# acg-team/ProGraphMSA

Hardware: AMD Instinct MI355X
Metric: DP cell-updates/sec (GCUPS) + wall-clock on 256 seqs × 1000 aa, WAG (higher is better)
Workload: dtype f32

## Files before the change

prographmsa_amd/csrc/pgm_align_kernels.h:

```cpp
#ifndef PGM_ALIGN_KERNELS_H_
#define PGM_ALIGN_KERNELS_H_

#include <hip/hip_runtime.h>
#include <math.h>
#include <type_traits>
#include "pgm_device.h"

#define PGM_NEG_INF (-INFINITY)

__device__ __forceinline__ float pgm_ls_log_add(float x, float add) {
    const float a = 2.44247459618085927548717403238913328776812604856113966238617812902399112761292613763080658235564f;
    const float b = -4.2040783745848554315883301529007786406310628696382695994938550046831869207082846248658671f;
    const float c = -0.72123729809042963774358701619456664388406302428056983119308906451199556380646306f;
    const uint32_t bits = __float_as_uint(x);
    const float e = (float)((int32_t)(bits >> 23) - 126);
    const float d = __uint_as_float(((bits << 9) >> 9) ^ 0x3f000000u);
    float t = __fdiv_rn(b, __fsub_rn(d, c));
    const float u = __fadd_rn(e, a);
    t = __fadd_rn(t, add);
    t = __fadd_rn(t, u);
    return t;
}

__device__ __forceinline__ float pgm_emission_finish(float num, float ay, float bx, float match_init) {
    float q = __fdiv_rn(num, __fmul_rn(ay, bx));
    if (q != q) q = __uint_as_float(0xFFC00000u);
    return pgm_ls_log_add(q, match_init);
}

template <int DMAX, int NODES>
__global__ void __launch_bounds__(NODES) pgm_prep_kernel(const PgmJob *__restrict__ jobs, int *__restrict__ sync, uint32_t sync_ints) {
    extern __shared__ float prep_lds[];
    {
        const uint32_t nthreads = gridDim.x * gridDim.y * gridDim.z * NODES;
        const uint32_t gid = ((blockIdx.z * gridDim.y + blockIdx.y) * gridDim.x + blockIdx.x) * NODES + threadIdx.x;
        for (uint32_t i = gid; i < sync_ints; i += nthreads) sync[i] = 0;
    }
    const PgmJob &J = jobs[blockIdx.x];
    const bool first = blockIdx.y == 0;
    const uint32_t n = first ? J.n1 : J.n2;
    const uint32_t v0 = blockIdx.z * NODES;
    if (v0 >= n) return;
    if (J.tabhdr && J.tabhdr[0] == 0) {
        const uint32_t nc = J.dim + 2u;
        bool any = n - 1u >= v0 && n - 1u < v0 + (uint32_t)NODES;
        for (uint32_t c = 0; c < nc; ++c) {
            const uint32_t r = (uint32_t)J.tabhdr[1u + (first ? 0u : nc) + c];
            any = any || (r != 0u && r - 1u >= v0 && r - 1u < v0 + (uint32_t)NODES);
        }
        if (!any) return;
    }
    const uint32_t D = J.dim, DP = J.dp, ST = D + 1;
    float *Mf = prep_lds;
    float *pif = prep_lds + D * D;
    float *nl = pif + D;
    const uint32_t nn = min((uint32_t)NODES, n - v0);
    {
        const int32_t *pp = first ? J.pp1 : J.pp2;
        const uint32_t *pc = first ? J.pc1 : J.pc2, *pu = first ? J.pu1 : J.pu2;
        const float *pv = first ? J.pv1 : J.pv2;
        PgmTbNode *rec = (first ? J.tb1 : J.tb2) + v0;
        for (uint32_t i = threadIdx.x; i < nn * PGM_TB_PK; i += NODES) {
            const uint32_t node = i / PGM_TB_PK, k = i % PGM_TB_PK;
            const int32_t eb = pp[v0 + node];
            const uint32_t cnt = (uint32_t)(pp[v0 + node + 1] - eb);
            const int32_t e = cnt == 0u ? 0 : eb + (int32_t)min(k, cnt - 1u);
            if (k == 0) rec[node].cnt = cnt;
            rec[node].c[k] = pc[e]; rec[node].v[k] = pv[e]; rec[node].u[k] = pu[e];
        }
    }
    if (!first) for (uint32_t i = threadIdx.x; i < D * D; i += NODES) Mf[i] = (float)J.M[i];
    for (uint32_t i = threadIdx.x; i < D; i += NODES) pif[i] = (float)J.pi[i];
    const double *sites = first ? J.sites1 : J.sites2;
    const uint32_t *smap = first ? J.smap1 : J.smap2;
    float *dst = (first ? J.g1f : J.t2) + (size_t)DP * v0;
    for (uint32_t i = threadIdx.x; i < nn * D; i += NODES) {
        const uint32_t node = v0 + i / D;
        const float g = (float)sites[(size_t)D * (smap ? smap[node] : node) + i % D];
        nl[(i / D) * ST + (i % D)] = g;
        if (first && DP == D) dst[i] = g;
    }
    __syncthreads();
    const uint32_t v = threadIdx.x;
    float g[DMAX];
    float acc = 0.0f;
    if (v < nn) {
#pragma unroll
        for (int k = 0; k < DMAX; ++k) g[k] = ((uint32_t)k < D) ? nl[v * ST + k] : 0.0f;
        float l0 = 0.0f, l1 = 0.0f, l2 = 0.0f, l3 = 0.0f;
        const uint32_t aligned = D / 4u * 4u;
#pragma unroll
        for (int k = 0; k + 3 < DMAX; k += 4) {
            if ((uint32_t)k < aligned) {
                l0 = __fadd_rn(l0, __fmul_rn(g[k], pif[k]));
                l1 = __fadd_rn(l1, __fmul_rn(g[k + 1], pif[k + 1]));
                l2 = __fadd_rn(l2, __fmul_rn(g[k + 2], pif[k + 2]));
                l3 = __fadd_rn(l3, __fmul_rn(g[k + 3], pif[k + 3]));
            }
        }
        acc = __fadd_rn(0.0f, __fadd_rn(__fadd_rn(l0, l2), __fadd_rn(l1, l3)));
#pragma unroll
        for (int k = 0; k < DMAX; ++k)
            if ((uint32_t)k >= aligned && (uint32_t)k < D) acc = __fadd_rn(acc, __fmul_rn(g[k], pif[k]));
        (first ? J.a1 : J.b2)[v0 + v] = acc;
    }
    if (first) {
        if (DP != D && v < nn) {
#pragma unroll
            for (int k = 0; k < DMAX; ++k) if ((uint32_t)k < DP) dst[(size_t)DP * v + k] = g[k];
        }
        return;
    }
    __syncthreads();
    if (v < nn) {
        for (uint32_t k = 0; k < D; ++k) {
            float t = 0.0f;
#pragma unroll
            for (int j = 0; j < DMAX; ++j)
                if ((uint32_t)j < D) t = __fadd_rn(t, __fmul_rn(Mf[j + D * k], g[j]));
            nl[v * ST + k] = t;
        }
    }
    __syncthreads();
    for (uint32_t i = threadIdx.x; i < nn * DP; i += NODES) {
        const uint32_t node = i / DP, k = i % DP;
        dst[i] = k < D ? nl[node * ST + k] : 0.0f;
    }
}

#define PGM_TAB_HDR 136
__global__ void __launch_bounds__(256) pgm_classify_kernel(const PgmJob *__restrict__ jobs) {
    const PgmJob &J = jobs[blockIdx.x];
    if (!J.tabhdr) return;
    const bool first = blockIdx.y == 0;
    const uint32_t n = first ? J.n1 : J.n2, D = J.dim;
    const double *sites = first ? J.sites1 : J.sites2;
    const uint32_t *smap = first ? J.smap1 : J.smap2;
    uint8_t *cls = (uint8_t *)(first ? J.cls1 : J.cls2);
    const float uni = (float)(1.0 / (double)D);
    for (uint32_t v = blockIdx.z * blockDim.x + threadIdx.x; v < n; v += gridDim.z * blockDim.x) {
        const double *col = sites + (size_t)D * (smap ? smap[v] : v);
        uint32_t nz = 0, sym = 0;
        bool same = true;
        float vs = 0.f;
        const float g0 = (float)col[0];
        for (uint32_t k = 0; k < D; ++k) {
            const float g = (float)col[k];
            if (g != 0.0f) { ++nz; sym = k; vs = g; }
            same = same && g == g0;
        }
        uint32_t c = 255u;
        if (nz == 0u) c = D + 1u;
        else if (nz == 1u && vs == 1.0f) c = sym;
        else if (same && g0 == uni) c = D;
        cls[v] = (uint8_t)c;
        if (c == 255u) atomicOr(J.tabhdr, 1);
        else atomicCAS(J.tabhdr + 1 + (first ? 0u : D + 2u) + c, 0, (int)v + 1);
    }
}

__device__ __forceinline__ size_t pgm_cell_index(const PgmJob &J, uint32_t y, uint32_t x) {
    const uint32_t b = y / PGM_ROWS, l = PGM_HALO + (y - b * PGM_ROWS);
    return ((size_t)b * J.tsteps + (x + l)) * 64u + l;
}
__device__ __forceinline__ float4 pgm_load_cell(const PgmJob &J, uint32_t y, uint32_t x) {
    return J.cells[pgm_cell_index(J, y, x)];
}

__device__ __forceinline__ float pgm_dpp_wave_shr1(float src, float lane0_value) {
    return __int_as_float(__builtin_amdgcn_update_dpp(__float_as_int(lane0_value), __float_as_int(src), 0x138, 0xf, 0xf, false));
}

#define PGM_GLOBAL __attribute__((address_space(1)))
typedef float pgm_v4f __attribute__((ext_vector_type(4)));
template <class T> __device__ __forceinline__ T pgm_gld(const T *p) { return *(const PGM_GLOBAL T *)(uintptr_t)p; }
#define PGM_EM_TB 4
template <int DP, int RB>
__global__ void __launch_bounds__(4 * PGM_ROWS) pgm_emission_skew_kernel(const PgmJob *__restrict__ jobs) {
    typedef float pgm_v2f __attribute__((ext_vector_type(2)));
    constexpr int NT = DP / 4;
    constexpr int COLS = 64 + PGM_EM_TB * PGM_BLOCK - PGM_HALO - 1;
    constexpr int STR = DP + 1;
    __shared__ pgm_v2f tp[(COLS + 1) * STR];
    __shared__ float bq[COLS];
    const PgmJob &J = jobs[blockIdx.z];
    const uint32_t tb0 = blockIdx.x * PGM_EM_TB;
    const uint32_t rsh = J.rshift, nvb = J.nb << rsh;
    if (tb0 >= J.nblk || 4u * RB * blockIdx.y >= nvb) return;
    if (J.tabhdr && pgm_gld(J.tabhdr) == 0) return;
    auto row_of = [&](uint32_t v, uint32_t lane_) { return ((((v >> rsh) << 6) + lane_) << rsh) | (v & ((1u << rsh) - 1u)); };
    auto sblock_of = [&](uint32_t v, uint32_t tb_) { return ((((size_t)(v >> rsh) * J.nblk + tb_) << rsh) | (v & ((1u << rsh) - 1u))); };
    const uint32_t t0 = tb0 * PGM_BLOCK;
    const int cbase = (int)t0 - 63;
    if ((DP == 20 || DP == 4) && RB == 1) {
        constexpr int TE = DP + 1;
        float *const tab = (float *)tp;
        static_assert(COLS * TE <= (COLS + 1) * STR * 2, "score table must fit the column staging area");
        static_assert(DP > 20 || TE <= 32, "row classes must fit As");
        __shared__ float As[32];
        const uint32_t fb0 = 4u * blockIdx.y + threadIdx.x / PGM_ROWS;
        const uint32_t fl = threadIdx.x % PGM_ROWS;
        const bool active = fb0 < nvb;
        int sym = DP;
        bool plain = true;
        float a_row = 0.f;
        if (active) {
            const uint32_t y = row_of(fb0, fl);
            const uint32_t yc = (y + 1 < J.n1) ? y : 0u;
            const float4 *src = (const float4 *)(J.g1f + (size_t)DP * yc);
            int nz = 0;
#pragma unroll
            for (int q = 0; q < NT; ++q) {
                const float4 v = src[q];
                const float vv[4] = {v.x, v.y, v.z, v.w};
#pragma unroll
                for (int u = 0; u < 4; ++u)
                    if (vv[u] != 0.0f) { ++nz; sym = 4 * q + u; plain = plain && vv[u] == 1.0f; }
            }
            plain = plain && nz <= 1;
            a_row = J.a1[yc];
        }
        if (threadIdx.x < 32) As[threadIdx.x] = 0.f;
        if (__syncthreads_and(plain ? 1 : 0)) {
            if (active) As[sym] = a_row;
            __syncthreads();
            const float mi = J.sc.match_init;
            constexpr int NE = (COLS * TE + 4 * PGM_ROWS - 1) / (4 * PGM_ROWS);
            float tt[NE], tb2[NE];
#pragma unroll
            for (int e = 0; e < NE; ++e) {
                const int i = (int)threadIdx.x + e * 4 * PGM_ROWS;
                const int ci = i / TE, k = i % TE, c = cbase + ci;
                const bool in = i < COLS * TE && c >= 0 && c <= (int)J.ncol;
                tb2[e] = in ? J.b2[c] : 0.f;
                tt[e] = (in && k < DP) ? J.t2[(size_t)DP * c + k] : 0.f;
            }
#pragma unroll
            for (int e = 0; e < NE; ++e) {
                const int i = (int)threadIdx.x + e * 4 * PGM_ROWS;
                if (i < COLS * TE) tab[i] = pgm_emission_finish(0.0f + tt[e], As[i % TE], tb2[e], mi);
            }
            __syncthreads();
            if (!active) return;
            PGM_GLOBAL pgm_v4f *const Sq = (PGM_GLOBAL pgm_v4f *)(uintptr_t)J.S;
            const int l = PGM_HALO + (int)fl;
#pragma unroll 1
            for (int w = 0; w < PGM_EM_TB; ++w) {
                const uint32_t tb = tb0 + w;
                if (tb >= J.nblk) break;
                float out[PGM_BLOCK];
#pragma unroll
                for (int i = 0; i < PGM_BLOCK; ++i) out[i] = tab[((int)(tb * PGM_BLOCK) + i - l - cbase) * TE + sym];
                PGM_GLOBAL pgm_v4f *dst = Sq + (sblock_of(fb0, tb) * 64u + (uint32_t)l) * (PGM_BLOCK / 4);
#pragma unroll
                for (int q = 0; q < PGM_BLOCK / 4; ++q) dst[q] = pgm_v4f{out[4 * q], out[4 * q + 1], out[4 * q + 2], out[4 * q + 3]};
            }
            return;
        }
    }
    const float4 *t2q = (const float4 *)J.t2;
    float *tpf = (float *)tp;
    for (int i = threadIdx.x; i < (COLS + 1) * NT; i += 4 * PGM_ROWS) {
        const int ci = i / NT, q = i % NT, c = cbase + ci;
        float4 v = make_float4(0.f, 0.f, 0.f, 0.f);
        if (c >= 0 && c <= (int)J.ncol) v = t2q[(size_t)NT * c + q];
        const float vv[4] = {v.x, v.y, v.z, v.w};
#pragma unroll
        for (int u = 0; u < 4; ++u) {
            const int k = 4 * q + u;
            if (ci < COLS) tpf[2 * (ci * STR + k)] = vv[u];
            if (ci > 0) tpf[2 * ((ci - 1) * STR + k) + 1] = vv[u];
        }
    }
    for (int i = threadIdx.x; i < COLS; i += 4 * PGM_ROWS) {
        const int col = cbase + i;
        bq[i] = (col >= 0 && col <= (int)J.ncol) ? J.b2[col] : 0.f;
    }
    __syncthreads();
    const uint32_t b0 = (4u * blockIdx.y + threadIdx.x / PGM_ROWS) * RB;
    const int l = PGM_HALO + (int)(threadIdx.x % PGM_ROWS);
    if (b0 >= nvb) return;
    float gy[RB][DP], ay[RB];
#pragma unroll
    for (int r = 0; r < RB; ++r) {
        const uint32_t y = row_of(b0 + (uint32_t)r, (uint32_t)(l - PGM_HALO));
        const uint32_t yc = (y + 1 < J.n1) ? y : 0u;
        const float4 *src = (const float4 *)(J.g1f + (size_t)DP * yc);
#pragma unroll
        for (int q = 0; q < NT; ++q) {
            const float4 v = src[q];
            gy[r][4 * q] = v.x; gy[r][4 * q + 1] = v.y; gy[r][4 * q + 2] = v.z; gy[r][4 * q + 3] = v.w;
        }
        ay[r] = J.a1[yc];
    }
    const float mi = J.sc.match_init;
    const uint32_t nblk = J.nblk;
    PGM_GLOBAL pgm_v4f *const Sq = (PGM_GLOBAL pgm_v4f *)(uintptr_t)J.S;
#pragma unroll 1
    for (int w = 0; w < PGM_EM_TB; ++w) {
        const uint32_t tb = tb0 + w;
        if (tb >= nblk) break;
        float out[RB][PGM_BLOCK];
#pragma unroll
        for (int i = 0; i < PGM_BLOCK; i += 2) {
            const int ci = (int)(tb * PGM_BLOCK) + i - l - cbase;
            const pgm_v2f *tc = tp + ci * STR;
            pgm_v2f acc[RB];
#pragma unroll
            for (int r = 0; r < RB; ++r) acc[r] = pgm_v2f{0.0f, 0.0f};
#pragma unroll
            for (int k = 0; k < DP; ++k) {
                const pgm_v2f tk = tc[k];
#pragma unroll
                for (int r = 0; r < RB; ++r) {
                    const pgm_v2f g = {gy[r][k], gy[r][k]};
                    acc[r] = acc[r] + g * tk;
                }
            }
#pragma unroll
            for (int r = 0; r < RB; ++r) {
                out[r][i] = pgm_emission_finish(acc[r].x, ay[r], bq[ci], mi);
                out[r][i + 1] = pgm_emission_finish(acc[r].y, ay[r], bq[ci + 1], mi);
            }
        }
#pragma unroll
        for (int r = 0; r < RB; ++r) {
            if (b0 + (uint32_t)r < nvb) {
                PGM_GLOBAL pgm_v4f *dst = Sq + (sblock_of(b0 + (uint32_t)r, tb) * 64u + (uint32_t)l) * (PGM_BLOCK / 4);
#pragma unroll
                for (int q = 0; q < PGM_BLOCK / 4; ++q) dst[q] = pgm_v4f{out[r][4 * q], out[r][4 * q + 1], out[r][4 * q + 2], out[r][4 * q + 3]};
            }
        }
// ... 2263 lines not shown
```

prographmsa_amd/csrc/pgm_capi.hip:

```cpp
#include <hip/hip_runtime.h>

#include <algorithm>
#include <cmath>
#include <cstdio>
#include <thread>
#include <atomic>
#include <chrono>
#include <queue>
#include <cstdlib>
#include <cstring>
#include <numeric>
#include <mutex>
#include <string>
#include <unordered_set>
#include <vector>
#include <sys/mman.h>

#include "pgm_align_kernels.h"
#include "pgm_crit_kernels.h"
#include "pgm_nw_kernels.h"
#include "pgm_csprofile_kernels.h"
#include "pgm_dist_kernels.h"
#include "pgm_merge_kernels.h"
#include "pgm_parsimony_kernels.h"
// ... 88 lines not shown
static hipError_t pinned_alloc(size_t bytes, void **out) {
    const size_t H = (size_t)2 << 20, len = (std::max<size_t>(bytes, 1) + H - 1) / H * H;
    void *p = getenv("PGM_PINNED_MALLOC") ? nullptr : aligned_alloc(H, len);
    if (p) {
        (void)madvise(p, len, MADV_HUGEPAGE);
        (void)lib_pool().run(len / H, len >= 8 * H ? 16u : 1u, [&](size_t c) { for (size_t o = 0; o < H; o += 4096) ((volatile char *)p)[c * H + o] = 0; });
        if (hipHostRegister(p, len, hipHostRegisterDefault) == hipSuccess) {
            std::lock_guard<std::mutex> g(g_pinned_mu);
            g_pinned_registered.insert(p);
            *out = p;
            return hipSuccess;
        }
        (void)hipGetLastError();
        free(p);
    }
    return hipHostMalloc(out, bytes, hipHostMallocDefault);
}
static void pinned_free(void *p) {
    if (!p) return;
    bool reg;
    { std::lock_guard<std::mutex> g(g_pinned_mu); reg = g_pinned_registered.erase(p) != 0; }
    if (reg) { (void)hipHostUnregister(p); free(p); }
    else (void)hipHostFree(p);
}
static void slot_free(int slot, void *p) {
    if (slot == pgm_ctx::C_HIN) pinned_free(p);
    else if (slot == pgm_ctx::C_HOST) (void)hipHostFree(p);
    else (void)hipFree(p);
}

struct pgm_align_batch {
    uint32_t njobs = 0;
    uint64_t cells = 0;
    uint32_t maxdim = 0, maxnb = 0, maxn = 0, maxnblk = 0;
    std::vector<PgmJob> jobs;
    std::vector<uint32_t> order;
    BatchSchedule sched;
    uint8_t *d_in = nullptr;
    uint8_t *d_work = nullptr;
    uint8_t *d_cells = nullptr;
    uint8_t *d_out = nullptr;
    uint8_t *d_S = nullptr;
    uint8_t *d_small = nullptr;
    size_t in_bytes = 0, work_bytes = 0, cell_bytes = 0, out_bytes = 0, s_bytes = 0, small_bytes = 0;
    size_t cap[8] = {0, 0, 0, 0, 0, 0, 0, 0};
    uint8_t *h_out = nullptr;
    uint8_t *h_in = nullptr;
    int *h_flag = nullptr;
    int *d_sync = nullptr;
    size_t sync_ints = 0;
    uint32_t lq_off = 0;
    PgmJob *d_jobs = nullptr;
    uint32_t *d_order = nullptr;
    PgmItem *d_items = nullptr;
    uint32_t *d_lean = nullptr;
    PgmItem *d_bands = nullptr;
    int2 *d_tblist = nullptr;
    unsigned long long *d_times = nullptr;
    int *d_tabhdr = nullptr;
    hipEvent_t ev_fork = nullptr, ev_join = nullptr;
    hipEvent_t ev_join_b = nullptr, ev_join_c = nullptr;
    uint32_t test_spin_limit = 0, test_stall_job = 0xFFFFFFFFu, test_stall_band = 0;
    double acc_ms[3] = {0, 0, 0};
    uint32_t acc_n = 0;
    bool ev_pending = false;
    std::vector<size_t> res_off, map1_off, map2_off;
    hipEvent_t ev[5] = {nullptr, nullptr, nullptr, nullptr, nullptr};
};
static const struct BatchBuffer { int slot; size_t reserve_mb; uint8_t *pgm_align_batch::*ptr; size_t pgm_align_batch::*bytes; } kBatchBuffers[6] = {
    {pgm_ctx::C_IN, 128, &pgm_align_batch::d_in, &pgm_align_batch::in_bytes}, {pgm_ctx::C_WORK, 256, &pgm_align_batch::d_work, &pgm_align_batch::work_bytes},
    {pgm_ctx::C_CELLS, 2048, &pgm_align_batch::d_cells, &pgm_align_batch::cell_bytes}, {pgm_ctx::C_OUT, 8, &pgm_align_batch::d_out, &pgm_align_batch::out_bytes},
    {pgm_ctx::C_S, 1024, &pgm_align_batch::d_S, &pgm_align_batch::s_bytes}, {pgm_ctx::C_SMALL, 4, &pgm_align_batch::d_small, &pgm_align_batch::small_bytes}};

extern "C" {

const char *pgm_last_error(void) { return g_err.c_str(); }

int pgm_device_count(void) {
    int n = 0;
    if (hipGetDeviceCount(&n) != hipSuccess) return 0;
    return n;
}

__global__ void pgm_warm_kernel() {}

int pgm_ctx_create(int device, pgm_ctx **out) {
    if (!out) return fail(PGM_ERR_INVALID, "null out");
    *out = nullptr;
    int n = 0;
    HIPCHK(hipGetDeviceCount(&n));
    if (device < 0 || device >= n) return fail(PGM_ERR_DEVICE, "no such HIP device");
    HIPCHK(hipSetDevice(device));
    pgm_ctx *c = new pgm_ctx;
    c->device = device;
    HIPCHK(hipGetDeviceProperties(&c->prop, device));
    HIPCHK(hipStreamCreateWithFlags(&c->stream, hipStreamNonBlocking));
    HIPCHK(hipStreamCreateWithFlags(&c->stream2, hipStreamNonBlocking));
    HIPCHK(hipStreamCreateWithFlags(&c->stream3, hipStreamNonBlocking));
    {
        int lo = 0, hi = 0;
        if (hipDeviceGetStreamPriorityRange(&lo, &hi) != hipSuccess) { (void)hipGetLastError(); lo = hi = 0; }
        if (hipStreamCreateWithPriority(&c->stream4, hipStreamNonBlocking, hi) != hipSuccess) {
            (void)hipGetLastError();
            HIPCHK(hipStreamCreateWithFlags(&c->stream4, hipStreamNonBlocking));
        }
    }
// ... 163 lines not shown
    void up(void *dst, const void *src, size_t bytes) { if (ok() && bytes) { queued = true; e = hipMemcpyAsync(dst, src, bytes, hipMemcpyHostToDevice, s); } }
    void zero(void *dst, size_t bytes) { if (ok() && bytes) { queued = true; e = hipMemsetAsync(dst, 0, bytes, s); } }
    void down(void *dst, const void *src, size_t bytes) { if (ok() && bytes) { queued = true; e = hipMemcpyAsync(dst, src, bytes, hipMemcpyDeviceToHost, s); } }
    void bufs(int first, int end, std::initializer_list<Buf> list) {
        if (ok() && (size_t)(end - first) < list.size()) e = hipErrorInvalidValue;
        for (const Buf &b : list) { buf(first++, b.bytes, b.p); if (b.src) up(*b.p, b.src, b.bytes); }
    }
    bool begin() {
        if (ok()) e = scratch_events(ctx);
        if (ok()) { queued = true; e = hipEventRecord(ctx->sc_ev[0], s); }
        return ok();
    }
    void end() {
        if (ok()) e = hipGetLastError();
        if (ok()) e = hipEventRecord(ctx->sc_ev[1], s);
        timed = ok();
    }
    int finish() {
        if (queued) { const hipError_t es = hipStreamSynchronize(s); if (ok()) e = es; }
        if (ok() && timed && ms) (void)hipEventElapsedTime(ms, ctx->sc_ev[0], ctx->sc_ev[1]);
        if (ok()) return PGM_OK;
        (void)hipGetLastError();
        return fail(alloc_failed && e == hipErrorOutOfMemory ? PGM_ERR_NOMEM : PGM_ERR_DEVICE, std::string(what) + ": " + hipGetErrorString(e));
    }
};

static hipError_t classify_lean_jobs(pgm_ctx *ctx, pgm_align_batch *b) {
    if (!b->d_tabhdr || b->njobs == 0) return hipSuccess;
    hipError_t e = hipMemsetAsync(b->d_tabhdr, 0, 4 * (size_t)PGM_TAB_HDR * b->njobs, ctx->stream);
    if (e != hipSuccess) return e;
    hipLaunchKernelGGL(pgm_classify_kernel, dim3(b->njobs, 2, (b->maxn + 1023) / 1024), dim3(256), 0, ctx->stream, b->d_jobs);
    return hipGetLastError();
}

#define PGM_STATUS_PENDING 0x7ffffff0
struct PrepTier { uint32_t tier, threads; size_t lds; };
static PrepTier prep_tier(uint32_t maxdim) {
    const uint32_t tier = alphabet_tier(maxdim), threads = tier == 64u ? 64u : 256u;
    return {tier, threads, ((size_t)maxdim * maxdim + maxdim + threads * ((size_t)maxdim + 1)) * sizeof(float)};
}
static hipError_t launch_all(pgm_ctx *ctx, pgm_align_batch *b, bool timed) {
    hipStream_t s = ctx->stream;
    const BatchSchedule &S = b->sched;
    hipError_t e;
    for (uint32_t i = 0; i < b->njobs; ++i) ((PgmJob::Result *)(b->h_out + b->res_off[i]))->status = PGM_STATUS_PENDING;
    if (timed && (e = hipEventRecord(b->ev[0], s)) != hipSuccess) return e;
    const PrepTier T = prep_tier(b->maxdim);
    const dim3 pg(b->njobs, 2, (b->maxn + T.threads - 1) / T.threads);
    if (T.tier == 4) hipLaunchKernelGGL((pgm_prep_kernel<4, 256>), pg, dim3(256), T.lds, s, b->d_jobs, b->d_sync, (uint32_t)b->sync_ints);
    else if (T.tier == 20) hipLaunchKernelGGL((pgm_prep_kernel<20, 256>), pg, dim3(256), T.lds, s, b->d_jobs, b->d_sync, (uint32_t)b->sync_ints);
    else hipLaunchKernelGGL((pgm_prep_kernel<64, 64>), pg, dim3(64), T.lds, s, b->d_jobs, b->d_sync, (uint32_t)b->sync_ints);
    if ((e = hipGetLastError()) != hipSuccess) return e;
    if (timed && (e = hipEventRecord(b->ev[1], s)) != hipSuccess) return e;
    const dim3 eg((b->maxnblk + PGM_EM_TB - 1) / PGM_EM_TB, (b->maxnb + 3) / 4, b->njobs);
    if (T.tier == 4) hipLaunchKernelGGL((pgm_emission_skew_kernel<4, 1>), eg, dim3(4 * PGM_ROWS), 0, s, b->d_jobs);
    else if (T.tier == 20) hipLaunchKernelGGL((pgm_emission_skew_kernel<20, 1>), eg, dim3(4 * PGM_ROWS), 0, s, b->d_jobs);
    else hipLaunchKernelGGL((pgm_emission_skew_kernel<64, 1>), eg, dim3(4 * PGM_ROWS), 0, s, b->d_jobs);
    if ((e = hipGetLastError()) != hipSuccess) return e;
    if (timed && (e = hipEventRecord(b->ev[2], s)) != hipSuccess) return e;
    const uint32_t spin_limit = b->test_spin_limit ? b->test_spin_limit : PGM_SPIN_LIMIT, stall_job = b->test_stall_job, stall_band = b->test_stall_band;
    const bool fork = S.nlean != 0;
    const bool bandk = S.nbands != 0;
    const bool tbk = (S.nitems != 0 || bandk) && (S.ntb + S.ntb_c + S.ntb_b) != 0;
    const bool critk = S.ncrit != 0;
    if ((fork || bandk || critk) && (e = hipEventRecord(b->ev_fork, s)) != hipSuccess) return e;
    if (critk && (e = hipStreamWaitEvent(ctx->stream4, b->ev_fork, 0)) != hipSuccess) return e;
    if (fork && (e = hipStreamWaitEvent(ctx->stream2, b->ev_fork, 0)) != hipSuccess) return e;
    if (bandk && (e = hipStreamWaitEvent(ctx->stream3, b->ev_fork, 0)) != hipSuccess) return e;
    const uint32_t nrest = S.nitems - S.ncrit;
    hipStream_t sc = critk ? s : ctx->stream4, sr = critk ? ctx->stream4 : s;
    auto sweep = [&](hipStream_t st, uint32_t workers, const PgmItem *list, uint32_t n, bool c3, uint32_t ticket_off) {
        if (c3) hipLaunchKernelGGL(pgm_crit_kernel, dim3(workers), dim3(64 * PGM_C3_WAVES), 0, st, b->d_jobs, list, n, b->d_sync, spin_limit, stall_job, stall_band, ticket_off);
        else hipLaunchKernelGGL(pgm_fill_kernel, dim3(workers), dim3(64 * PGM_WAVES), 0, st, b->d_jobs, list, n, b->d_sync, spin_limit, stall_job, stall_band, ticket_off);
    };
    auto tracebacks = [&](hipStream_t st, uint32_t workers, uint32_t first, uint32_t n, uint32_t lq_off, uint32_t sybase) {
        hipLaunchKernelGGL(pgm_tb_kernel, dim3(workers), dim3(64 * PGM_WAVES), 0, st, b->d_jobs, b->d_tblist + first, n, b->d_sync, b->test_spin_limit, lq_off, sybase, 1u);
    };
    if (critk) sweep(sc, S.ncrit_workers, b->d_items, S.ncrit, S.crit_c3, (uint32_t)PGM_SY_CRIT_TICKET);
    if (nrest != 0) sweep(sr, S.nworkers, b->d_items + S.ncrit, nrest, S.rest_c3, 1u);
    if ((e = hipGetLastError()) != hipSuccess) return e;
    if (fork) {
        hipLaunchKernelGGL((pgm_lean_kernel<2>), dim3(S.nlean_workers), dim3(64 * PGM_WAVES), 0, ctx->stream2, b->d_jobs, b->d_lean, S.nlean, b->d_sync, spin_limit);
        if ((e = hipGetLastError()) != hipSuccess) return e;
    }
    const uint32_t njp = (b->njobs + 3u) / 4u * 4u;
    if (bandk) {
        hipLaunchKernelGGL(pgm_band_kernel, dim3(S.nband_workers), dim3(64 * PGM_WAVES), 0, ctx->stream3, b->d_jobs, b->d_bands, S.nbands_narrow, S.nbands, S.nband_workers - S.nwide_workers, b->d_sync, spin_limit, stall_job, stall_band);
        if ((e = hipGetLastError()) != hipSuccess) return e;
        if (tbk && S.ntb_b) tracebacks(ctx->stream3, S.ntb_b_workers, S.ntb + S.ntb_c, S.ntb_b, b->lq_off + njp, 8u);
        if ((e = hipGetLastError()) != hipSuccess) return e;
        if ((e = hipEventRecord(b->ev_join_b, ctx->stream3)) != hipSuccess) return e;
    }
    if (critk) {
        if (tbk && S.ntb_c) tracebacks(sc, S.ncrit_workers, S.ntb, S.ntb_c, b->lq_off + 2 * njp, 16u);
        if ((e = hipGetLastError()) != hipSuccess) return e;
    }
    if (tbk && S.ntb) {
        tracebacks(sr, S.ntb_workers, 0u, S.ntb, b->lq_off, 0u);
        if ((e = hipGetLastError()) != hipSuccess) return e;
    }
    if (critk && (e = hipEventRecord(b->ev_join_c, ctx->stream4)) != hipSuccess) return e;
    if (bandk && (e = hipStreamWaitEvent(s, b->ev_join_b, 0)) != hipSuccess) return e;
    if (critk && (e = hipStreamWaitEvent(s, b->ev_join_c, 0)) != hipSuccess) return e;
    if (fork && ((e = hipEventRecord(b->ev_join, ctx->stream2)) != hipSuccess || (e = hipStreamWaitEvent(s, b->ev_join, 0)) != hipSuccess)) return e;
    if (timed && (e = hipEventRecord(b->ev[3], s)) != hipSuccess) return e;
    if (timed && (e = hipEventRecord(b->ev[4], s)) != hipSuccess) return e;
    return hipSuccess;
}
struct SmallLayout { size_t sync, jobs, order, items, lean, tblist, bands, times, tabhdr, total_bands; bool any_lean; };
static SmallLayout layout_small(pgm_align_batch *b) {
    SmallLayout s;
    const uint32_t njobs = b->njobs;
    s.total_bands = 0; s.any_lean = false;
    for (const PgmJob &J : b->jobs) { s.total_bands += J.nb; s.any_lean = s.any_lean || (J.lean && !J.keep_cells); }
    DevLayout SM;
    s.sync = SM.take(b->sync_ints * sizeof(int)); s.jobs = SM.take(sizeof(PgmJob) * std::max(1u, njobs));
    s.order = SM.take(4 * (size_t)std::max(1u, njobs)); s.items = SM.take(sizeof(PgmItem) * std::max<size_t>(1, s.total_bands));
    s.lean = SM.take(4 * (size_t)std::max(1u, njobs)); s.tblist = SM.take(8 * (size_t)std::max(1u, njobs));
    s.bands = SM.take(sizeof(PgmItem) * std::max<size_t>(1, s.total_bands)); s.times = SM.take(16 * (size_t)std::max(1u, njobs) + 16);
    s.tabhdr = SM.take(s.any_lean ? 4 * (size_t)PGM_TAB_HDR * njobs : 16);
    b->small_bytes = SM.bytes;
    return s;
}

static double now_ms() { return std::chrono::duration<double, std::milli>(std::chrono::steady_clock::now().time_since_epoch()).count(); }

struct BatchAlloc {
    std::atomic<int> state{0};
    hipError_t err = hipSuccess, host_err = hipSuccess;
    uint8_t *h_out_dev = nullptr;
    double ms_dev = 0, ms_host = 0, ms_slot[6] = {0, 0, 0, 0, 0, 0};
};
static void take_batch_buffers(pgm_ctx *ctx, pgm_align_batch *b, SmallLayout sm, BatchAlloc *A) {
    const double ta0 = now_ms();
    hipError_t e2 = hipSetDevice(ctx->device);
    double tprev = ta0;
    for (int k = 0; k < 6 && e2 == hipSuccess; ++k) {
        const BatchBuffer &s = kBatchBuffers[k];
        e2 = cache_take(ctx, s.slot, b->*s.bytes, (void **)&(b->*s.ptr), &b->cap[s.slot]);
        const double t = now_ms(); A->ms_slot[k] = t - tprev; tprev = t;
    }
    if (e2 == hipSuccess) {
        b->d_sync = (int *)(b->d_small + sm.sync);
        b->d_jobs = (PgmJob *)(b->d_small + sm.jobs);
        b->d_order = (uint32_t *)(b->d_small + sm.order);
        b->d_items = (PgmItem *)(b->d_small + sm.items);
        b->d_lean = (uint32_t *)(b->d_small + sm.lean);
        b->d_tblist = (int2 *)(b->d_small + sm.tblist);
        b->d_bands = (PgmItem *)(b->d_small + sm.bands);
        b->d_times = (unsigned long long *)(b->d_small + sm.times);
        b->d_tabhdr = sm.any_lean ? (int *)(b->d_small + sm.tabhdr) : nullptr;
    }
    A->err = e2;
    A->state.store(e2 == hipSuccess ? 1 : -1, std::memory_order_release);
    A->ms_dev = now_ms() - ta0;
    if (e2 == hipSuccess) {
        hipError_t e3 = cache_take(ctx, pgm_ctx::C_HOST, b->out_bytes + 64, (void **)&b->h_out, &b->cap[pgm_ctx::C_HOST]);
        if (e3 == hipSuccess) b->h_flag = (int *)(b->h_out + (b->out_bytes + 15) / 16 * 16);
        if (e3 == hipSuccess) e3 = hipHostGetDevicePointer((void **)&A->h_out_dev, b->h_out, 0);
        A->host_err = e3;
    }
    A->ms_host = now_ms() - ta0 - A->ms_dev;
}

struct CreateGuard {
    pgm_ctx *ctx;
    pgm_align_batch *b;
    std::thread alloc;
    ~CreateGuard() { if (alloc.joinable()) alloc.join(); if (b) pgm_align_batch_destroy(ctx, b); }
    pgm_align_batch *release() { pgm_align_batch *r = b; b = nullptr; return r; }
};

static void bind_job_pointers(pgm_align_batch *b, const std::vector<JobOff> &off, const pgm_site_ref *res1, const pgm_site_ref *res2, uint8_t *h_out_dev) {
    for (uint32_t i = 0; i < b->njobs; ++i) {
        PgmJob &J = b->jobs[i];
        const JobOff &o = off[i];
        uint8_t *in = b->d_in, *w = b->d_work, *ob = b->d_out;
        J.sites1 = site_ref_of(res1, i) ? res1[i].dev_sites : (const double *)(in + o.s1.sites);
        J.sites2 = site_ref_of(res2, i) ? res2[i].dev_sites : (const double *)(in + o.s2.sites);
        J.smap1 = o.s1.has_smap ? (const uint32_t *)(in + o.s1.smap) : nullptr;
        J.smap2 = o.s2.has_smap ? (const uint32_t *)(in + o.s2.smap) : nullptr;
        J.M = (const double *)(in + o.M); J.pi = (const double *)(in + o.pi);
        J.ni1 = (const PgmNode2 *)(in + o.s1.ni); J.ni2 = (const PgmNode2 *)(in + o.s2.ni);
        J.xp1 = (const int32_t *)(in + o.s1.xp); J.xp2 = (const int32_t *)(in + o.s2.xp);
        J.xc1 = (const uint32_t *)(in + o.s1.xc); J.xc2 = (const uint32_t *)(in + o.s2.xc);
        J.xv1 = (const float *)(in + o.s1.xv); J.xv2 = (const float *)(in + o.s2.xv);
        J.fp1 = (const int32_t *)(in + o.s1.fp); J.fe1 = (const uint2 *)(in + o.s1.fe);
        J.ov2 = (const uint2 *)(in + o.s2.ov);
        J.pp1 = (const int32_t *)(in + o.s1.pp); J.pp2 = (const int32_t *)(in + o.s2.pp);
        J.pc1 = (const uint32_t *)(in + o.s1.pc); J.pc2 = (const uint32_t *)(in + o.s2.pc);
        J.pv1 = (const float *)(in + o.s1.pv); J.pv2 = (const float *)(in + o.s2.pv);
        J.pu1 = (const uint32_t *)(in + o.s1.pu); J.pu2 = (const uint32_t *)(in + o.s2.pu);
        J.g1f = (float *)(w + o.g1f); J.a1 = (float *)(w + o.a1);
        J.t2 = (float *)(w + o.t2); J.b2 = (float *)(w + o.aux2);
        J.map1 = (uint32_t *)(ob + o.map1); J.map2 = (uint32_t *)(ob + o.map2);
        J.mark_score = (float *)(w + o.ms); J.mark_prev = (uint32_t *)(w + o.mp);
        J.tb1 = (PgmTbNode *)(w + o.tb1); J.tb2 = (PgmTbNode *)(w + o.tb2);
        J.result = (PgmJob::Result *)(ob + o.res);
        J.hmap1 = (uint32_t *)(h_out_dev + o.map1); J.hmap2 = (uint32_t *)(h_out_dev + o.map2);
        J.hresult = (PgmJob::Result *)(h_out_dev + o.res);
        J.cells = (float4 *)(b->d_cells + o.cells);
        J.codes = (uint32_t *)(w + o.codes);
        J.endcell = (float4 *)(w + o.endcell);
        if (J.lean && !J.keep_cells && b->d_tabhdr) { J.cls1 = w + o.cls; J.cls2 = w + o.cls + J.n1; J.tabhdr = b->d_tabhdr + (size_t)PGM_TAB_HDR * i; }
// ... 80 lines not shown
    CreateGuard G{ctx, new pgm_align_batch, {}};
    pgm_align_batch *b = G.b;
    b->njobs = njobs;
    std::vector<char> two_chains(njobs, 0);
    (void)lib_pool().run(njobs, njobs >= 16 ? 16u : 1u, [&](size_t i) { two_chains[i] = job_is_two_chains(g1[i], g2[i]) ? 1 : 0; });
    BatchSizes Z;
    const int invalid = plan_sizes(njobs, g1, g2, model, scores, flags, res1, res2, two_chains, cus, b->jobs, Z);
    if (invalid >= 0) return fail(PGM_ERR_INVALID, "invalid job " + std::to_string(invalid));
    const std::vector<size_t> &in_base = Z.in_base;
    b->maxdim = Z.maxdim; b->maxnb = Z.maxnb; b->maxn = Z.maxn; b->maxnblk = Z.maxnblk; b->cells = Z.cells;
    b->res_off.resize(njobs); b->map1_off.resize(njobs); b->map2_off.resize(njobs);
    for (uint32_t i = 0; i < njobs; ++i) { b->res_off[i] = Z.off[i].res; b->map1_off[i] = Z.off[i].map1; b->map2_off[i] = Z.off[i].map2; }
    b->in_bytes = std::max<size_t>(in_base[njobs], 16);
    b->work_bytes = std::max<size_t>(Z.L.W.bytes, 16);
    b->cell_bytes = std::max<size_t>(Z.L.C.bytes, 16);
    b->out_bytes = std::max<size_t>(Z.L.O.bytes, 16);
    b->s_bytes = std::max<size_t>(Z.L.SL.bytes, 16);
    b->lq_off = (uint32_t)Z.L.sync_ints;
    b->sync_ints = Z.L.sync_ints + 3 * (((size_t)njobs + 3) / 4 * 4);
    const double tc0 = now_ms();
    const SmallLayout sm = layout_small(b);
    G.alloc = std::thread(take_batch_buffers, ctx, b, sm, &A);
    hipError_t e;
    if ((e = cache_take(ctx, pgm_ctx::C_HIN, b->in_bytes, (void **)&b->h_in, &b->cap[pgm_ctx::C_HIN])) != hipSuccess)
        return fail(PGM_ERR_DEVICE, std::string("hipHostMalloc: ") + hipGetErrorString(e));
    const double tc1 = now_ms();
    std::atomic<int> bad(-1), upload_err((int)hipSuccess);
    const uint32_t chunk_jobs = (uint32_t)std::max<size_t>(1, ((size_t)8 << 20) / std::max<size_t>(1, in_base[njobs] / std::max(1u, njobs)));
    std::vector<std::atomic<uint32_t>> chunk_done((njobs + chunk_jobs - 1) / chunk_jobs + 1);
    for (auto &cd : chunk_done) cd.store(0);
    (void)lib_pool().run(njobs, 16, [&](size_t job_index) {
        const uint32_t i = (uint32_t)job_index;
        if (!plan_flatten_job(b->h_in, in_base[i], in_base[i + 1], g1[i], g2[i], model[i], site_ref_of(res1, i), site_ref_of(res2, i), Z.pro, b->jobs[i], Z.off[i])) { bad.store((int)i); return; }
        const uint32_t c = i / chunk_jobs, c0 = c * chunk_jobs, c1 = std::min(njobs, c0 + chunk_jobs);
        if (chunk_done[c].fetch_add(1, std::memory_order_acq_rel) + 1 == c1 - c0) {
            int st;
            while ((st = A.state.load(std::memory_order_acquire)) == 0) std::this_thread::yield();
            if (st == 1) {
                (void)hipSetDevice(ctx->device);
                const hipError_t eu = hipMemcpyAsync(b->d_in + in_base[c0], b->h_in + in_base[c0], in_base[c1] - in_base[c0], hipMemcpyHostToDevice, ctx->stream);
                if (eu != hipSuccess) upload_err.store((int)eu);
            }
        }
    });
    if (bad.load() >= 0) return fail(PGM_ERR_INVALID, "invalid graph in job " + std::to_string(bad.load()));
    const double tc2 = now_ms();
    G.alloc.join();
    const double tc3 = now_ms();
    if (A.err != hipSuccess) return fail(A.err == hipErrorOutOfMemory ? PGM_ERR_NOMEM : PGM_ERR_DEVICE, std::string("hipMalloc: ") + hipGetErrorString(A.err));
    if (A.host_err != hipSuccess) return fail(PGM_ERR_DEVICE, std::string("hipHostMalloc: ") + hipGetErrorString(A.host_err));
    bind_job_pointers(b, Z.off, res1, res2, A.h_out_dev);
    b->order = size_order(b->jobs);
    b->sched = plan_schedule(b->jobs, b->order, cus);
    const BatchSchedule &S = b->sched;
    if (cprof && njobs)
        fprintf(stderr, "    work lists: longest chain of sweeps %.0f us, goal %.0f us; lean %zu jobs %.0f us-worker on %u CUs; bands %zu, %.0f us-worker on %u CUs (simulated end %.0f us); items %zu, %.0f us-worker on %u CUs (simulated end %.0f us), of the longest chains %zu on %u CUs (%.0f us)\n",
                S.rsweep, S.t_goal, (size_t)S.nlean, S.lean_cost, S.nlean_workers, S.total_b, S.band_cost, S.nband_workers, S.band_end, S.total, S.other_cost, S.capacity, S.fill_end, S.total_c, S.ncrit_workers, S.crit_end);
    const double tc4 = now_ms();
    if (S.nitems > std::max<size_t>(1, sm.total_bands)) return fail(PGM_ERR_DEVICE, "work list longer than the number of bands");
    if ((e = (hipError_t)upload_err.load()) != hipSuccess ||
        (e = hipMemcpyAsync(b->d_tblist, S.tblist.data(), 8 * S.tblist.size(), hipMemcpyHostToDevice, ctx->stream)) != hipSuccess ||
        (e = hipMemcpyAsync(b->d_jobs, b->jobs.data(), sizeof(PgmJob) * njobs, hipMemcpyHostToDevice, ctx->stream)) != hipSuccess ||
        (e = hipMemcpyAsync(b->d_order, b->order.data(), 4 * (size_t)njobs, hipMemcpyHostToDevice, ctx->stream)) != hipSuccess ||
        (e = hipMemcpyAsync(b->d_items, S.items.data(), sizeof(PgmItem) * S.items.size(), hipMemcpyHostToDevice, ctx->stream)) != hipSuccess ||
        (e = hipMemcpyAsync(b->d_lean, S.lean_list.data(), 4 * S.lean_list.size(), hipMemcpyHostToDevice, ctx->stream)) != hipSuccess ||
        (e = hipMemcpyAsync(b->d_bands, S.bands.data(), sizeof(PgmItem) * S.bands.size(), hipMemcpyHostToDevice, ctx->stream)) != hipSuccess ||
        (e = classify_lean_jobs(ctx, b)) != hipSuccess ||
        (e = hipStreamSynchronize(ctx->stream)) != hipSuccess)
        return fail(PGM_ERR_DEVICE, std::string("upload: ") + hipGetErrorString(e));
    for (int k = 0; k < 5; ++k) (void)hipEventCreate(&b->ev[k]);
    (void)hipEventCreateWithFlags(&b->ev_fork, hipEventDisableTiming);
    (void)hipEventCreateWithFlags(&b->ev_join, hipEventDisableTiming);
    (void)hipEventCreateWithFlags(&b->ev_join_b, hipEventDisableTiming);
    (void)hipEventCreateWithFlags(&b->ev_join_c, hipEventDisableTiming);
    if (cprof)
        fprintf(stderr, "    create: sizes %.2f ms, pinned input block %.2f, flatten %.2f, wait for the allocations %.2f (device %.2f, pinned results %.2f), work list %.2f, upload of %.1f MB %.2f\n",
                tc0 - tcs, tc1 - tc0, tc2 - tc1, tc3 - tc2, A.ms_dev, A.ms_host, tc4 - tc3, b->in_bytes / 1e6, now_ms() - tc4);
    if (cprof)
        fprintf(stderr, "    device buffers: inputs %.1f MB %.2f ms, work %.1f MB %.2f, cells %.1f MB %.2f, results %.1f MB %.2f, S %.1f MB %.2f, small %.2f\n",
                b->in_bytes / 1e6, A.ms_slot[0], b->work_bytes / 1e6, A.ms_slot[1], b->cell_bytes / 1e6, A.ms_slot[2], b->out_bytes / 1e6, A.ms_slot[3], b->s_bytes / 1e6, A.ms_slot[4], A.ms_slot[5]);
    *out = G.release();
    return PGM_OK;
}

int pgm_align_batch_run(pgm_ctx *ctx, pgm_align_batch *b) {
    if (!ctx || !b) return fail(PGM_ERR_INVALID, "null argument");
    if (b->njobs == 0) return PGM_OK;
    HIPCHK(hipSetDevice(ctx->device));
    HIPCHK(launch_all(ctx, b, true));
    b->ev_pending = true;
    return PGM_OK;
}

int pgm_align_batch_time(pgm_ctx *ctx, pgm_align_batch *b, int reps, float *ms_prep, float *ms_emission, float *ms_fill,
                         float *ms_traceback) {
    if (!ctx || !b || reps <= 0) return fail(PGM_ERR_INVALID, "bad argument");
    HIPCHK(hipSetDevice(ctx->device));
    double acc[4] = {0, 0, 0, 0};
    for (int r = 0; r < reps && b->njobs; ++r) {
        HIPCHK(launch_all(ctx, b, true));
        b->ev_pending = false;
        HIPCHK(hipEventSynchronize(b->ev[4]));
        for (int k = 0; k < 4; ++k) {
            float ms = 0;
            HIPCHK(hipEventElapsedTime(&ms, b->ev[k], b->ev[k + 1]));
            acc[k] += ms;
        }
    }
    if (ms_prep) *ms_prep = (float)(acc[0] / reps);
    if (ms_emission) *ms_emission = (float)(acc[1] / reps);
    if (ms_fill) *ms_fill = (float)(acc[2] / reps);
    if (ms_traceback) *ms_traceback = (float)(acc[3] / reps);
    return PGM_OK;
}

int pgm_align_batch_job_times(pgm_ctx *ctx, pgm_align_batch *b, uint64_t *ticks) {
// ... 200 lines not shown
```

Baseline: 80.64.

## Compact emission grid per job and unroll prep kernel gathers for memory parallelism

The emission kernel no longer launches a padded 3D grid sized to the largest job. It launches a flat 1D grid built from a per-job prefix table, and each workgroup finds its job with a binary search, so workgroups that would exit at once for small jobs are never created. The prep kernel's gather loops are also unrolled eight ways, issuing all index and value loads before the stores to raise memory-level parallelism. The cost is an extra table upload, a binary search per workgroup, and more registers in the prep kernel.

```diff
diff --git a/prographmsa_amd/csrc/pgm_align_kernels.h b/prographmsa_amd/csrc/pgm_align_kernels.h
--- a/prographmsa_amd/csrc/pgm_align_kernels.h
+++ b/prographmsa_amd/csrc/pgm_align_kernels.h
@@ -5,6 +5,7 @@
 #include <math.h>
 #include <type_traits>
 #include "pgm_device.h"
+#include "pgm_grid.h"
 
 #define PGM_NEG_INF (-INFINITY)
 
@@ -28,6 +29,7 @@
     return pgm_ls_log_add(q, match_init);
 }
 
+#define PGM_PREP_U 8
 template <int DMAX, int NODES>
 __global__ void __launch_bounds__(NODES) pgm_prep_kernel(const PgmJob *__restrict__ jobs, int *__restrict__ sync, uint32_t sync_ints) {
     extern __shared__ float prep_lds[];
@@ -60,13 +62,31 @@
         const uint32_t *pc = first ? J.pc1 : J.pc2, *pu = first ? J.pu1 : J.pu2;
         const float *pv = first ? J.pv1 : J.pv2;
         PgmTbNode *rec = (first ? J.tb1 : J.tb2) + v0;
-        for (uint32_t i = threadIdx.x; i < nn * PGM_TB_PK; i += NODES) {
-            const uint32_t node = i / PGM_TB_PK, k = i % PGM_TB_PK;
-            const int32_t eb = pp[v0 + node];
-            const uint32_t cnt = (uint32_t)(pp[v0 + node + 1] - eb);
-            const int32_t e = cnt == 0u ? 0 : eb + (int32_t)min(k, cnt - 1u);
-            if (k == 0) rec[node].cnt = cnt;
-            rec[node].c[k] = pc[e]; rec[node].v[k] = pv[e]; rec[node].u[k] = pu[e];
+        const uint32_t nrec = nn * PGM_TB_PK;
+        for (uint32_t i0 = threadIdx.x; i0 < nrec; i0 += NODES * PGM_PREP_U) {
+            int32_t eb[PGM_PREP_U], ee[PGM_PREP_U];
+#pragma unroll
+            for (int u = 0; u < PGM_PREP_U; ++u) {
+                const uint32_t node = min(i0 + (uint32_t)u * NODES, nrec - 1u) / PGM_TB_PK;
+                eb[u] = pp[v0 + node]; ee[u] = pp[v0 + node + 1];
+            }
+            uint32_t rc[PGM_PREP_U], ru[PGM_PREP_U];
+            float rv[PGM_PREP_U];
+#pragma unroll
+            for (int u = 0; u < PGM_PREP_U; ++u) {
+                const uint32_t k = min(i0 + (uint32_t)u * NODES, nrec - 1u) % PGM_TB_PK, cnt = (uint32_t)(ee[u] - eb[u]);
+                const int32_t e = cnt == 0u ? 0 : eb[u] + (int32_t)min(k, cnt - 1u);
+                rc[u] = pc[e]; rv[u] = pv[e]; ru[u] = pu[e];
+            }
+#pragma unroll
+            for (int u = 0; u < PGM_PREP_U; ++u) {
+                const uint32_t i = i0 + (uint32_t)u * NODES;
+                if (i < nrec) {
+                    const uint32_t node = i / PGM_TB_PK, k = i % PGM_TB_PK;
+                    if (k == 0) rec[node].cnt = (uint32_t)(ee[u] - eb[u]);
+                    rec[node].c[k] = rc[u]; rec[node].v[k] = rv[u]; rec[node].u[k] = ru[u];
+                }
+            }
         }
     }
     if (!first) for (uint32_t i = threadIdx.x; i < D * D; i += NODES) Mf[i] = (float)J.M[i];
@@ -74,11 +94,25 @@
     const double *sites = first ? J.sites1 : J.sites2;
     const uint32_t *smap = first ? J.smap1 : J.smap2;
     float *dst = (first ? J.g1f : J.t2) + (size_t)DP * v0;
-    for (uint32_t i = threadIdx.x; i < nn * D; i += NODES) {
-        const uint32_t node = v0 + i / D;
-        const float g = (float)sites[(size_t)D * (smap ? smap[node] : node) + i % D];
-        nl[(i / D) * ST + (i % D)] = g;
-        if (first && DP == D) dst[i] = g;
+    const uint32_t nval = nn * D;
+    for (uint32_t i0 = threadIdx.x; i0 < nval; i0 += NODES * PGM_PREP_U) {
+        uint32_t col[PGM_PREP_U];
+#pragma unroll
+        for (int u = 0; u < PGM_PREP_U; ++u) {
+            const uint32_t node = v0 + min(i0 + (uint32_t)u * NODES, nval - 1u) / D;
+            col[u] = smap ? smap[node] : node;
+        }
+        float g[PGM_PREP_U];
+#pragma unroll
+        for (int u = 0; u < PGM_PREP_U; ++u) g[u] = (float)sites[(size_t)D * col[u] + min(i0 + (uint32_t)u * NODES, nval - 1u) % D];
+#pragma unroll
+        for (int u = 0; u < PGM_PREP_U; ++u) {
+            const uint32_t i = i0 + (uint32_t)u * NODES;
+            if (i < nval) {
+                nl[(i / D) * ST + (i % D)] = g[u];
+                if (first && DP == D) dst[i] = g[u];
+            }
+        }
     }
     __syncthreads();
     const uint32_t v = threadIdx.x;
@@ -175,18 +209,23 @@
 typedef float pgm_v4f __attribute__((ext_vector_type(4)));
 template <class T> __device__ __forceinline__ T pgm_gld(const T *p) { return *(const PGM_GLOBAL T *)(uintptr_t)p; }
 #define PGM_EM_TB 4
+static_assert(PGM_EM_TB == PGM_GRID_EM_TB && PGM_GRID_EM_BANDS == 4u, "pgm_grid.h lays out the emission kernel's workgroups");
 template <int DP, int RB>
-__global__ void __launch_bounds__(4 * PGM_ROWS) pgm_emission_skew_kernel(const PgmJob *__restrict__ jobs) {
+__global__ void __launch_bounds__(4 * PGM_ROWS) pgm_emission_skew_kernel(const PgmJob *__restrict__ jobs, const uint32_t *__restrict__ gfirst, uint32_t njobs) {
     typedef float pgm_v2f __attribute__((ext_vector_type(2)));
     constexpr int NT = DP / 4;
     constexpr int COLS = 64 + PGM_EM_TB * PGM_BLOCK - PGM_HALO - 1;
     constexpr int STR = DP + 1;
     __shared__ pgm_v2f tp[(COLS + 1) * STR];
     __shared__ float bq[COLS];
-    const PgmJob &J = jobs[blockIdx.z];
-    const uint32_t tb0 = blockIdx.x * PGM_EM_TB;
+    static_assert(RB == 1, "pgm_grid.h counts four bands per workgroup");
+    const uint32_t job = pgm_grid_find(gfirst, njobs, blockIdx.x);
+    const PgmJob &J = jobs[job];
+    const uint32_t wg = blockIdx.x - gfirst[job], gx = pgm_grid_em_x(J.nblk);
+    const uint32_t bx = wg % gx, by = wg / gx;
+    const uint32_t tb0 = bx * PGM_EM_TB;
     const uint32_t rsh = J.rshift, nvb = J.nb << rsh;
-    if (tb0 >= J.nblk || 4u * RB * blockIdx.y >= nvb) return;
+    if (tb0 >= J.nblk || 4u * RB * by >= nvb) return;
     if (J.tabhdr && pgm_gld(J.tabhdr) == 0) return;
     auto row_of = [&](uint32_t v, uint32_t lane_) { return ((((v >> rsh) << 6) + lane_) << rsh) | (v & ((1u << rsh) - 1u)); };
     auto sblock_of = [&](uint32_t v, uint32_t tb_) { return ((((size_t)(v >> rsh) * J.nblk + tb_) << rsh) | (v & ((1u << rsh) - 1u))); };
@@ -198,7 +237,7 @@
         static_assert(COLS * TE <= (COLS + 1) * STR * 2, "score table must fit the column staging area");
         static_assert(DP > 20 || TE <= 32, "row classes must fit As");
         __shared__ float As[32];
-        const uint32_t fb0 = 4u * blockIdx.y + threadIdx.x / PGM_ROWS;
+        const uint32_t fb0 = 4u * by + threadIdx.x / PGM_ROWS;
         const uint32_t fl = threadIdx.x % PGM_ROWS;
         const bool active = fb0 < nvb;
         int sym = DP;
@@ -277,7 +316,7 @@
         bq[i] = (col >= 0 && col <= (int)J.ncol) ? J.b2[col] : 0.f;
     }
     __syncthreads();
-    const uint32_t b0 = (4u * blockIdx.y + threadIdx.x / PGM_ROWS) * RB;
+    const uint32_t b0 = (4u * by + threadIdx.x / PGM_ROWS) * RB;
     const int l = PGM_HALO + (int)(threadIdx.x % PGM_ROWS);
     if (b0 >= nvb) return;
     float gy[RB][DP], ay[RB];
diff --git a/prographmsa_amd/csrc/pgm_capi.hip b/prographmsa_amd/csrc/pgm_capi.hip
--- a/prographmsa_amd/csrc/pgm_capi.hip
+++ b/prographmsa_amd/csrc/pgm_capi.hip
@@ -164,6 +164,8 @@
     uint32_t lq_off = 0;
     PgmJob *d_jobs = nullptr;
     uint32_t *d_order = nullptr;
+    PgmGridTable grid;
+    uint32_t *d_grid_em = nullptr;
     PgmItem *d_items = nullptr;
     uint32_t *d_lean = nullptr;
     PgmItem *d_bands = nullptr;
@@ -433,10 +435,10 @@
     else hipLaunchKernelGGL((pgm_prep_kernel<64, 64>), pg, dim3(64), T.lds, s, b->d_jobs, b->d_sync, (uint32_t)b->sync_ints);
     if ((e = hipGetLastError()) != hipSuccess) return e;
     if (timed && (e = hipEventRecord(b->ev[1], s)) != hipSuccess) return e;
-    const dim3 eg((b->maxnblk + PGM_EM_TB - 1) / PGM_EM_TB, (b->maxnb + 3) / 4, b->njobs);
-    if (T.tier == 4) hipLaunchKernelGGL((pgm_emission_skew_kernel<4, 1>), eg, dim3(4 * PGM_ROWS), 0, s, b->d_jobs);
-    else if (T.tier == 20) hipLaunchKernelGGL((pgm_emission_skew_kernel<20, 1>), eg, dim3(4 * PGM_ROWS), 0, s, b->d_jobs);
-    else hipLaunchKernelGGL((pgm_emission_skew_kernel<64, 1>), eg, dim3(4 * PGM_ROWS), 0, s, b->d_jobs);
+    const dim3 eg(b->grid.em_total());
+    if (T.tier == 4) hipLaunchKernelGGL((pgm_emission_skew_kernel<4, 1>), eg, dim3(4 * PGM_ROWS), 0, s, b->d_jobs, b->d_grid_em, b->njobs);
+    else if (T.tier == 20) hipLaunchKernelGGL((pgm_emission_skew_kernel<20, 1>), eg, dim3(4 * PGM_ROWS), 0, s, b->d_jobs, b->d_grid_em, b->njobs);
+    else hipLaunchKernelGGL((pgm_emission_skew_kernel<64, 1>), eg, dim3(4 * PGM_ROWS), 0, s, b->d_jobs, b->d_grid_em, b->njobs);
     if ((e = hipGetLastError()) != hipSuccess) return e;
     if (timed && (e = hipEventRecord(b->ev[2], s)) != hipSuccess) return e;
     const uint32_t spin_limit = b->test_spin_limit ? b->test_spin_limit : PGM_SPIN_LIMIT, stall_job = b->test_stall_job, stall_band = b->test_stall_band;
@@ -488,7 +490,7 @@
     if (timed && (e = hipEventRecord(b->ev[4], s)) != hipSuccess) return e;
     return hipSuccess;
 }
-struct SmallLayout { size_t sync, jobs, order, items, lean, tblist, bands, times, tabhdr, total_bands; bool any_lean; };
+struct SmallLayout { size_t sync, jobs, order, items, lean, tblist, bands, times, tabhdr, grid_em, total_bands; bool any_lean; };
 static SmallLayout layout_small(pgm_align_batch *b) {
     SmallLayout s;
     const uint32_t njobs = b->njobs;
@@ -500,6 +502,7 @@
     s.lean = SM.take(4 * (size_t)std::max(1u, njobs)); s.tblist = SM.take(8 * (size_t)std::max(1u, njobs));
     s.bands = SM.take(sizeof(PgmItem) * std::max<size_t>(1, s.total_bands)); s.times = SM.take(16 * (size_t)std::max(1u, njobs) + 16);
     s.tabhdr = SM.take(s.any_lean ? 4 * (size_t)PGM_TAB_HDR * njobs : 16);
+    s.grid_em = SM.take(4 * ((size_t)njobs + 1));
     b->small_bytes = SM.bytes;
     return s;
 }
@@ -531,6 +534,7 @@
         b->d_bands = (PgmItem *)(b->d_small + sm.bands);
         b->d_times = (unsigned long long *)(b->d_small + sm.times);
         b->d_tabhdr = sm.any_lean ? (int *)(b->d_small + sm.tabhdr) : nullptr;
+        b->d_grid_em = (uint32_t *)(b->d_small + sm.grid_em);
     }
     A->err = e2;
     A->state.store(e2 == hipSuccess ? 1 : -1, std::memory_order_release);
@@ -717,6 +721,11 @@
     bind_job_pointers(b, Z.off, res1, res2, A.h_out_dev);
     b->order = size_order(b->jobs);
     b->sched = plan_schedule(b->jobs, b->order, cus);
+    {
+        std::vector<PgmGridJob> gj(njobs);
+        for (uint32_t k = 0; k < njobs; ++k) { const PgmJob &J = b->jobs[k]; gj[k] = PgmGridJob{J.nblk, J.nb << J.rshift}; }
+        if (!pgm_grid_build(gj, b->grid)) return fail(PGM_ERR_INVALID, "batch too large for one launch of the emission kernel");
+    }
     const BatchSchedule &S = b->sched;
     if (cprof && njobs)
         fprintf(stderr, "    work lists: longest chain of sweeps %.0f us, goal %.0f us; lean %zu jobs %.0f us-worker on %u CUs; bands %zu, %.0f us-worker on %u CUs (simulated end %.0f us); items %zu, %.0f us-worker on %u CUs (simulated end %.0f us), of the longest chains %zu on %u CUs (%.0f us)\n",
@@ -727,6 +736,7 @@
         (e = hipMemcpyAsync(b->d_tblist, S.tblist.data(), 8 * S.tblist.size(), hipMemcpyHostToDevice, ctx->stream)) != hipSuccess ||
         (e = hipMemcpyAsync(b->d_jobs, b->jobs.data(), sizeof(PgmJob) * njobs, hipMemcpyHostToDevice, ctx->stream)) != hipSuccess ||
         (e = hipMemcpyAsync(b->d_order, b->order.data(), 4 * (size_t)njobs, hipMemcpyHostToDevice, ctx->stream)) != hipSuccess ||
+        (e = hipMemcpyAsync(b->d_grid_em, b->grid.em.data(), 4 * b->grid.em.size(), hipMemcpyHostToDevice, ctx->stream)) != hipSuccess ||
         (e = hipMemcpyAsync(b->d_items, S.items.data(), sizeof(PgmItem) * S.items.size(), hipMemcpyHostToDevice, ctx->stream)) != hipSuccess ||
         (e = hipMemcpyAsync(b->d_lean, S.lean_list.data(), 4 * S.lean_list.size(), hipMemcpyHostToDevice, ctx->stream)) != hipSuccess ||
         (e = hipMemcpyAsync(b->d_bands, S.bands.data(), sizeof(PgmItem) * S.bands.size(), hipMemcpyHostToDevice, ctx->stream)) != hipSuccess ||
diff --git a/prographmsa_amd/csrc/pgm_grid.h b/prographmsa_amd/csrc/pgm_grid.h
--- /dev/null
+++ b/prographmsa_amd/csrc/pgm_grid.h
@@ -0,0 +1,45 @@
+#ifndef PGM_GRID_H_
+#define PGM_GRID_H_
+
+#include <stdint.h>
+#include <vector>
+
+#if defined(__HIPCC__)
+#define PGM_GRID_HD __host__ __device__ __forceinline__
+#else
+#define PGM_GRID_HD inline
+#endif
+
+#define PGM_GRID_EM_TB 4u
+#define PGM_GRID_EM_BANDS 4u
+#define PGM_GRID_MAX 0x7fffffffu
+
+PGM_GRID_HD uint32_t pgm_grid_find(const uint32_t *first, uint32_t n, uint32_t idx) {
+    uint32_t lo = 0, hi = n;
+    while (hi - lo > 1u) {
+        const uint32_t mid = lo + (hi - lo) / 2u;
+        if (first[mid] <= idx) lo = mid; else hi = mid;
+    }
+    return lo;
+}
+
+PGM_GRID_HD uint32_t pgm_grid_em_x(uint32_t nblk) { return (nblk + PGM_GRID_EM_TB - 1u) / PGM_GRID_EM_TB; }
+PGM_GRID_HD uint32_t pgm_grid_em_y(uint32_t nvb) { return (nvb + PGM_GRID_EM_BANDS - 1u) / PGM_GRID_EM_BANDS; }
+
+struct PgmGridJob { uint32_t nblk, nvb; };
+struct PgmGridTable {
+    std::vector<uint32_t> em;
+    uint32_t em_total() const { return em.back(); }
+};
+inline bool pgm_grid_build(const std::vector<PgmGridJob> &jobs, PgmGridTable &T) {
+    T.em.assign(1, 0u);
+    uint64_t e = 0;
+    for (const PgmGridJob &j : jobs) {
+        e += (uint64_t)pgm_grid_em_x(j.nblk) * pgm_grid_em_y(j.nvb);
+        if (e > PGM_GRID_MAX) return false;
+        T.em.push_back((uint32_t)e);
+    }
+    return true;
+}
+
+#endif
```

After: 81.85, median of 6. 1.01x the previous value.
